# tiems90/mosaic

Hardware: AMD Instinct MI355X
Metric: PIP-join points/sec (H3 res 9) at 1/2/4/8 GPUs + achieved HBM GB/s (higher is better)
Workload: dtype f64

## Files before the change

mosaic_amd/csrc/kernels.hip:

```cpp
#include <hip/hip_runtime.h>
#include <stdint.h>
#include <type_traits>

#include <map>
#include <mutex>

#define H3T_QUAL static __constant__ const
#include "h3_core.h"
#include "bng_core.h"
#include "pip_core.h"
#include "h3_ring.h"
#include "kernels.h"
#include "raster.h"

namespace mgpu {

#ifndef MGPU_BLOCK
#define MGPU_BLOCK 64
#endif
constexpr int kBlock = MGPU_BLOCK;
constexpr int kItems = 4;
constexpr int kTile = kBlock * kItems;
constexpr int kStreamBlock = 256;
static_assert(kTile <= 1024, "point-in-tile indices are 10 bits");
// ... 813 lines not shown
        const double2 q = s_cand_xy[point_stash<G>() ? (uint32_t)li : c];
        px = q.x;
        py = q.y;
      } else {
        px = a.x[MGPU_PT(li)];
        py = a.y[MGPU_PT(li)];
      }
      const ChipHdr& H = t.chip_hdr[ch];
      const uint32_t strip = H.strip_base + (uint32_t)strip_of(py, H.env[1], H.inv_h, (int)H.n_strips);
      one = H.single_ring != 0;
      fl = H.flags;
      pip::strip_bits(t, strip, one, px, py, sub * MGPU_EDGE_STEP, MGPU_EDGE_STEP << lg, &bnd, &par);
    }
    for (uint32_t o = 1; o < (1u << lg); o <<= 1) {
      bnd |= (uint32_t)__shfl_xor((int)bnd, (int)o);
      par ^= (uint32_t)__shfl_xor((int)par, (int)o);
    }
    if (m < nmix && sub == 0 && pip::strip_verdict(t, ch, one, fl, bnd, par, px, py))
      atomicOr(&s_mask[li], 1u << (pj >> 10));
  } else
#endif
  for (uint32_t m = threadIdx.x; m < nmix; m += kBlock) {
    const uint32_t c = s_mix[m];
    const uint32_t pj = s_cand_pj[c];
    const int li = pj & 1023;
    const uint32_t ch = s_first[li] + (pj >> 10);
    const int64_t p = MGPU_PT(li);
    double px, py;
    if (point_stash<G>() || c < (uint32_t)kStash) {
      const double2 q = s_cand_xy[point_stash<G>() ? (uint32_t)li : c];
      px = q.x;
      py = q.y;
    } else {
      px = a.x[p];
      py = a.y[p];
    }
    bool hit;
    if (SLOW && (t.chip_hdr[ch].flags & kChipNoStrips)) {
      hit = pip::chip_locate(t, ch, px, py) == pip::kInterior;
    } else {
#ifdef MGPU_STATS
      uint32_t ne = 0;
      hit = pip::chip_contains_mixed(t, ch, px, py, &ne);
      st_edges += ne;
#else
      hit = pip::chip_contains_mixed(t, ch, px, py);
#endif
    }
    if (hit) atomicOr(&s_mask[li], 1u << (pj >> 10));
  }
  }
#ifdef MGPU_STATS
  if (threadIdx.x == 0) {
    atomicAdd(&a.counters[8], (unsigned long long)s_nmix);
  }
  atomicAdd(&a.counters[9], (unsigned long long)st_edges);
#endif
  __syncthreads();

  MGPU_STAMP(3);
  if (G) {
    uint64_t v[kItems];
    uint32_t mine[kItems];
#pragma unroll
    for (int k = 0; k < kItems; k++) {
      const uint32_t li = threadIdx.x + k * kBlock;
      v[k] = 0;
      mine[k] = 0;
      if (li < gcount) {
        const uint32_t m = s_mask[li];
        v[k] = (uint64_t)s_first[li] | ((uint64_t)m << 32);
        if (a.poly_answers && m && !(m & (m - 1)))
          v[k] = (uint64_t)(uint32_t)t.chip_poly[s_first[li] + __builtin_ctz(m)] | (1ull << 32);
        mine[k] = __popc(m);
      }
    }
#pragma unroll
    for (int k = 0; k < kItems; k++) {
      const uint32_t li = threadIdx.x + k * kBlock;
      if (li < gcount) a.mixed_res[lbase + li] = v[k];
    }
    if (G == 1 && a.in_chunk_pairs) {
      const int lane = threadIdx.x & 63;
      const uint32_t s0 = 4u * (uint32_t)lane;
      const uint4 mq = *(const uint4*)(s_mask + s0);
      const uint32_t mv[4] = {mq.x, mq.y, mq.z, mq.w};
      uint32_t c[4], loc[4], nn[4];
#pragma unroll
      for (int i = 0; i < 4; i++) {
        const bool act = s0 + i < gcount;
        c[i] = act ? ckp[i] / (uint32_t)kChunk : 0xFFFFFFFFu;
        nn[i] = act ? (uint32_t)__popc(mv[i]) : 0u;
        loc[i] = (i ? loc[i - 1] : 0u) + nn[i];
      }
      const uint32_t lane_excl = wave_incl_scan(loc[3]) - loc[3];
      const uint32_t prev_c = __shfl_up(c[3], 1, 64), next_c = __shfl_down(c[0], 1, 64);
      bool head[4];
      uint32_t hpre = 0;
#pragma unroll
      for (int i = 0; i < 4; i++) {
        head[i] = c[i] != 0xFFFFFFFFu && (i ? c[i] != c[i - 1] : (lane == 0 || prev_c != c[0]));
        if (head[i]) hpre = lane_excl + loc[i] - nn[i];
      }
      const unsigned long long hl = __ballot(head[0] || head[1] || head[2] || head[3]);
      const unsigned long long lower = hl & ((1ull << lane) - 1ull);
      uint32_t start = __shfl(hpre, lower ? 63 - __clzll(lower) : 0, 64);
#pragma unroll
      for (int i = 0; i < 4; i++) {
        if (head[i]) start = lane_excl + loc[i] - nn[i];
        const bool tail = c[i] != 0xFFFFFFFFu && (i < 3 ? c[i + 1] != c[i] : (lane == 63 || next_c != c[3]));
        const uint32_t run = lane_excl + loc[i] - start;
        if (tail && run) atomicAdd(&a.in_chunk_pairs[c[i]], run);
      }
    }
    uint32_t tm = 0;
#pragma unroll
    for (int k = 0; k < kItems; k++) tm += mine[k];
    const unsigned long long tot = wave_sum_u64(tm);
    if ((threadIdx.x & 63) == 0 && tot) atomicAdd(&a.group_sum[chunk], (uint32_t)tot);
    return;
  }
  const int l0 = threadIdx.x * kItems;
  uint32_t mine = 0;
#pragma unroll
  for (int k = 0; k < kItems; k++) {
    const int li = l0 + k;
    mine += __popc(s_mask[li]);
    const uint32_t cnt = s_cnt[li];
    if (SLOW && cnt > (uint32_t)kMaskBits) {
      const int64_t p = MGPU_PT(li);
      const Range r{s_first[li], cnt, 0};
      for (uint32_t j = kMaskBits; j < cnt; j++)
        mine += (chip_is_core(t, r, j) || pip::chip_contains_strips(t, r.first + j, a.x[p], a.y[p])) ? 1 : 0;
    }
  }
  const int lane = threadIdx.x & 63, wave = threadIdx.x >> 6;
  uint32_t incl = wave_incl_scan(mine);
  if (lane == 63) s_wave_tot[wave] = incl;
  __syncthreads();
  uint32_t wave_off = 0, agg = 0;
#pragma unroll
  for (int w = 0; w < kBlock / 64; w++) {
    uint32_t v = s_wave_tot[w];
    if (w < wave) wave_off += v;
    agg += v;
  }
  const uint32_t excl = wave_off + incl - mine;

  __shared__ uint64_t s_dst;
  if (threadIdx.x == 0) {
    uint64_t dst = (uint64_t)tile * kSlot;
    if (agg > (uint32_t)kSlot) {
      const unsigned long long off = atomicAdd(a.pool_used, (unsigned long long)agg);
      dst = off + agg <= (unsigned long long)a.pool_cap ? (uint64_t)a.n_tiles * kSlot + off : kNoDst;
    }
    a.tile_count[tile] = agg;
    a.tile_where[tile] = dst;
    if (agg) atomicAdd(&a.group_sum[tile / kScanGroup], agg);
    s_dst = dst;
  }
  const bool staged = agg <= (uint32_t)kOutCap;
  __syncthreads();
  const uint64_t dst = s_dst;
  uint64_t* const rec = dst == kNoDst ? nullptr : a.recs + dst;

  uint32_t pos = excl;
#pragma unroll 1
  for (int k = 0; k < kItems; k++) {
    const int li = l0 + k;
    if (!SLOW) {
      const uint32_t first = s_first[li];
      for (uint32_t m = s_mask[li]; m; m &= m - 1) {
        const int32_t poly = t.chip_poly[first + __builtin_ctz(m)];
        if (staged) {
          s_out_poly[pos] = poly;
          s_out_li[pos] = (uint16_t)li;
        } else if (rec) {
          rec[pos] = ((uint64_t)li << 32) | (uint32_t)poly;
        }
        pos++;
      }
      continue;
    }
    const uint32_t cnt = s_cnt[li];
    if (!cnt) continue;
    const uint32_t first = s_first[li];
    const int64_t p = MGPU_PT(li);
    uint32_t m = s_mask[li];
    const uint32_t nj = cnt < (uint32_t)kMaskBits ? cnt : (uint32_t)kMaskBits;
    for (uint32_t j = 0; j < cnt; j++) {
      bool hit;
      if (!SLOW || j < nj) {
        hit = (m >> j) & 1;
      } else {
        const Range r{first, cnt, 0};
        hit = chip_is_core(t, r, j) || pip::chip_contains_strips(t, first + j, a.x[p], a.y[p]);
      }
      if (!hit) continue;
      const int32_t poly = t.chip_poly[first + j];
      if (staged) {
        s_out_poly[pos] = poly;
        s_out_li[pos] = (uint16_t)li;
      } else if (rec) {
        rec[pos] = ((uint64_t)li << 32) | (uint32_t)poly;
      }
      pos++;
    }
  }
  MGPU_STAMP(4);
  if (!staged || !rec) return;
  __syncthreads();
#ifndef MGPU_NT_RECS
#define MGPU_NT_RECS 1
#endif
  for (uint32_t i = threadIdx.x; i < agg; i += kBlock) {
    const uint64_t v = ((uint64_t)s_out_li[i] << 32) | (uint32_t)s_out_poly[i];
#if MGPU_NT_RECS
    __builtin_nontemporal_store(v, &rec[i]);
#else
    rec[i] = v;
#endif
  }
  MGPU_STAMP(4);
}

#ifndef MGPU_WAVES_PER_EU
#define MGPU_WAVES_PER_EU 8
#endif
#if MGPU_WAVES_PER_EU
#define MGPU_JOIN_ATTR __attribute__((amdgpu_waves_per_eu(MGPU_WAVES_PER_EU)))
#else
#define MGPU_JOIN_ATTR
#endif
template <int IS>
__global__ __launch_bounds__(kBlock) MGPU_JOIN_ATTR void pip_join_kernel(JoinArgs a) {
  join_tile<IS, false>(a, blockIdx.x);
}

template <int IS>
__global__ __launch_bounds__(kBlock) void pip_fix_kernel(JoinArgs a) {
  const uint32_t nd = *a.n_dirty;
  for (uint32_t q = blockIdx.x; q < nd; q += gridDim.x) {
    join_tile<IS, true>(a, a.dirty[q]);
    __syncthreads();
  }
}

#ifndef MGPU_CLS_BLOCK
#define MGPU_CLS_BLOCK 256
#endif
constexpr int kClsBlock = MGPU_CLS_BLOCK;
constexpr int kClsItems = kChunk / kClsBlock;
static_assert(kClsItems * (kClsBlock / 64) == 64, "one wave scans a chunk's ballots");
constexpr uint32_t kCodeMixed32 = 0xFFFFFFFFu;

template <int IS>
struct CodeOf {
  using T = uint16_t;
};
template <>
struct CodeOf<MGPU_BNG> {
  using T = uint32_t;
};


__device__ __forceinline__ uint32_t bng_grid_class(const JoinArgs& a, int64_t p, double px, double py, bool* ok,
                                                     uint32_t* first) {
  const ChipTableView& t = a.chips;
  bool tie = false;
  uint32_t gi = kNoEntry;
  Range r = chip_probe<MGPU_BNG, false>(a, p, px, py, ok, &tie, &gi);
  if (!*ok) return kPixEmpty;
  uint64_t e = 0;
  if (gi != kNoEntry) {
    e = t.grid[gi];
    r = grid_range(e, t.cell_ans_row != nullptr);
  }
  *first = r.first;
  if (r.count == 0) return kPixEmpty;
  if (r.count <= 8 && (r.core & ((1u << r.count) - 1u)) == (1u << r.count) - 1u) return (1u << r.count) - 1u;
  if (t.cell_ans_row && (e & kCellAnsFlag)) {
    const uint32_t eI = (uint32_t)bng::d2i(px), nI = (uint32_t)bng::d2i(py), ed = t.bng_edge;
    const uint32_t col = div_fix(eI, ed, t.bng_inv_edge), row = div_fix(nI, ed, t.bng_inv_edge);
    const uint32_t u = div_fix(eI - col * ed, t.cell_ans_sw, t.cell_ans_inv_sw);
    const uint32_t v = div_fix(nI - row * ed, t.cell_ans_sw, t.cell_ans_inv_sw);
    const uint32_t ai = t.cell_ans_row[row - (uint32_t)t.dense[0].b0] + cell_ans_index(e);
    const uint16_t m = t.cell_ans[((size_t)ai * t.cell_ans_g + v) * t.cell_ans_g + u];
    if (m != kCellAnsMixed && m < 256u) return m;
  }
  return kPixMixed;
}

#ifndef MGPU_CFY_BLOCK
#define MGPU_CFY_BLOCK 512
#endif
constexpr int kCfyBlock = MGPU_CFY_BLOCK;
#ifndef MGPU_CFY_BATCH
#define MGPU_CFY_BATCH 4
#endif
#ifndef MGPU_CFY_WAVES
#define MGPU_CFY_WAVES 1
#endif
constexpr int kCfyBatch = MGPU_CFY_BATCH;
template <int IS>
__global__ __launch_bounds__(kCfyBlock) __attribute__((amdgpu_waves_per_eu(MGPU_CFY_WAVES))) void classify_wave_kernel(SplitArgs sa, int64_t n_chunks) {
  using Code = typename CodeOf<IS>::T;
  constexpr int kW = kCfyBlock / 64;
  constexpr int kItems = kChunk / 64;
  static_assert(kItems % kCfyBatch == 0, "MGPU_CFY_BATCH must divide the points per lane of a chunk");
  const JoinArgs& a = sa.j;
  const ChipTableView& t = a.chips;
  extern __shared__ uint16_t s_blk[];
  const int lane = threadIdx.x & 63, wave = threadIdx.x >> 6;
  const bool use_blk = IS == MGPU_H3 && t.raster_blk != nullptr;
  const bool bng_grid = IS == MGPU_BNG && t.raster_mode == kRasterNone;
  const uint32_t nblk = use_blk ? t.raster_bnx * t.raster_bny : 0u;
  uint32_t* s_band = (uint32_t*)(s_blk + ((nblk + 1) & ~1u));
  if (use_blk)
    for (uint32_t i = threadIdx.x; i < nblk; i += kCfyBlock) s_blk[i] = t.raster_blk[i];
  if (IS == MGPU_H3)
    for (uint32_t i = threadIdx.x; i < t.raster_nband; i += kCfyBlock) s_band[i] = t.raster_band[i];
  __syncthreads();
  Code* codes = (Code*)sa.codes;
  const unsigned long long below = (1ull << lane) - 1ull;
  bool any_bad = false;
  const int64_t ch_step = (int64_t)gridDim.x * kW;
  double bx[kCfyBatch], by[kCfyBatch];
  auto load_batch = [&](int64_t ch, int b, double* X, double* Y) {
#pragma unroll
    for (int k = 0; k < kCfyBatch; k++) {
      const int64_t p = ch * kChunk + (int64_t)(b + k) * 64 + lane;
      X[k] = Y[k] = 0.0;
      if (ch < n_chunks && p < a.n) {
        X[k] = __builtin_nontemporal_load(&a.x[p]);
        Y[k] = __builtin_nontemporal_load(&a.y[p]);
      }
    }
  };
  for (int64_t ch = (int64_t)blockIdx.x * kW + wave; ch < n_chunks; ch += ch_step) {
    const int64_t c0 = ch * kChunk;
    uint32_t pairs = 0, nmixed = 0;
    for (int b = 0; b < kItems; b += kCfyBatch) {
      load_batch(ch, b, bx, by);
      uint32_t ri[kCfyBatch], gix[kCfyBatch], sb[kCfyBatch], bi[kCfyBatch];
#pragma unroll
      for (int k = 0; k < kCfyBatch; k++) {
        ri[k] = kNoPixel;
        gix[k] = 0;
        sb[k] = 0;
        bi[k] = kNoPixel;
        const int64_t pk = c0 + (int64_t)(b + k) * 64 + lane;
        if (pk < a.n && pt_valid(a.valid, a.valid_off, pk)) {
          bool ok = true;
          uint32_t g_ = 0, s_ = 0, b_ = kNoPixel;
          if (IS == MGPU_BNG && bng_grid) {
            const uint32_t m = bng_grid_class(a, pk, bx[k], by[k], &ok, &g_);
            ri[k] = m == kPixMixed ? kRasterFull : m;
          } else {
            ri[k] = raster_index<IS>(t, bx[k], by[k], &ok, &g_, &s_, &b_);
          }
          gix[k] = g_;
          sb[k] = s_;
          bi[k] = use_blk ? b_ : kNoPixel;
          any_bad |= !ok;
        }
      }
      uint32_t cl[kCfyBatch];
      uint64_t ge[kCfyBatch];
#ifndef MGPU_CFY_ABLATE
#define MGPU_CFY_ABLATE 0
#endif
#pragma unroll
      for (int k = 0; k < kCfyBatch; k++) {
#if MGPU_CFY_ABLATE == 1
        cl[k] = ri[k] < kRasterFull ? (ri[k] & 1) : kPixEmpty;
#elif MGPU_CFY_ABLATE == 2
        cl[k] = ri[k] < kRasterFull && bi[k] != kNoPixel && s_blk[bi[k]] != kPixMixed ? s_blk[bi[k]] : kPixEmpty;
#elif MGPU_CFY_ABLATE == 3
        cl[k] = ri[k] < kRasterFull ? (bi[k] != kNoPixel && s_blk[bi[k]] != kPixMixed ? s_blk[bi[k]] : t.raster[ri[k]])
                                    : kPixEmpty;
#elif MGPU_CFY_ABLATE == 4
        cl[k] = ri[k] < kRasterFull ? t.raster[ri[k]] : kPixEmpty;
#elif MGPU_CFY_ABLATE == 5
        cl[k] = ri[k] < kRasterFull ? (bi[k] != kNoPixel && s_blk[bi[k]] != kPixMixed ? s_blk[bi[k]] : kPixMixed)
                                    : kPixEmpty;
#else
        if (IS == MGPU_BNG && bng_grid)
          cl[k] = ri[k] == kRasterFull ? kPixMixed : (ri[k] == kNoPixel ? kPixEmpty : ri[k]);
        else
          cl[k] = ri[k] < kRasterFull ? raster_class_blk(t, s_blk, ri[k], bi[k], sb[k], s_band)
                                      : (ri[k] == kRasterFull ? kPixMixed : kPixEmpty);
#endif
        if (IS == MGPU_BNG && bng_grid) ge[k] = gix[k];
        else ge[k] = (IS == MGPU_BNG && ri[k] < kRasterFull) ? t.grid[gix[k]] : 0ull;
      }
#pragma unroll
      for (int k = 0; k < kCfyBatch; k++) {
        const int64_t p = c0 + (int64_t)(b + k) * 64 + lane;
        const bool valid = p < a.n;
        bool mixed = cl[k] == kPixMixed;
        Code code;
        if (IS == MGPU_H3) {
          code = (Code)cl[k];
          if (!mixed && cl[k] != kPixEmpty) {
            const uint32_t c = cl[k];
            pairs += c < t.raster_pc[0] ? 1u : c < t.raster_pc[1] ? 2u : c < t.raster_pc[2] ? 3u : c < t.raster_pc[3] ? 4u
                     : (uint32_t)__popc((uint32_t)(t.raster_cls[c] >> 32));
          }
        } else {
          const uint32_t first = (uint32_t)ge[k], m = cl[k];
          if (!mixed && m && !(m < 256u && first < (1u << 24))) mixed = true;
          code = (Code)(mixed ? kCodeMixed32 : (m ? (first << 8) | m : 0u));
          if (!mixed) pairs += __popc(m);
        }
        if (valid) MGPU_ST_INTER(code, &codes[p]);
        mixed = mixed && valid;
        const unsigned long long bal = __ballot(mixed);
        if (mixed) sa.mixed_idx[c0 + nmixed + (uint32_t)__popcll(bal & below)] = (uint16_t)((b + k) * 64 + lane);
        nmixed += (uint32_t)__popcll(bal);
      }
    }
    pairs = wave_sum_u32(pairs);
    if (lane == 0) {
      sa.chunk_pairs[ch] = pairs;
      sa.chunk_mixed[ch] = nmixed;
      a.group_cand[ch] = 0;
    }
  }
  count_wave(&a.counters[2], any_bad);
}


#ifndef MGPU_CFY_PAIR
#define MGPU_CFY_PAIR 1
#endif
typedef double dbl2_t __attribute__((ext_vector_type(2)));
template <int IS>
__global__ __launch_bounds__(kCfyBlock) __attribute__((amdgpu_waves_per_eu(MGPU_CFY_WAVES))) void classify_pair_kernel(SplitArgs sa, int64_t n_chunks) {
  using Code = typename CodeOf<IS>::T;
  constexpr int kW = kCfyBlock / 64;
  constexpr int kPairItems = kChunk / 128;
  constexpr int kPB = kCfyBatch / 2 > 0 ? kCfyBatch / 2 : 1;
  constexpr int kPts = 2 * kPB;
  static_assert(kPairItems % kPB == 0, "MGPU_CFY_BATCH / 2 must divide the pair items per lane of a chunk");
  const JoinArgs& a = sa.j;
  const ChipTableView& t = a.chips;
  extern __shared__ uint16_t s_blk[];
  const int lane = threadIdx.x & 63, wave = threadIdx.x >> 6;
  const bool use_blk = IS == MGPU_H3 && t.raster_blk != nullptr;
  const bool bng_grid = IS == MGPU_BNG && t.raster_mode == kRasterNone;
  const uint32_t nblk = use_blk ? t.raster_bnx * t.raster_bny : 0u;
  uint32_t* s_band = (uint32_t*)(s_blk + ((nblk + 1) & ~1u));
  if (use_blk)
    for (uint32_t i = threadIdx.x; i < nblk; i += kCfyBlock) s_blk[i] = t.raster_blk[i];
  if (IS == MGPU_H3)
    for (uint32_t i = threadIdx.x; i < t.raster_nband; i += kCfyBlock) s_band[i] = t.raster_band[i];
  __syncthreads();
  Code* codes = (Code*)sa.codes;
  const unsigned long long below = (1ull << lane) - 1ull;
  bool any_bad = false;
  const int64_t ch_step = (int64_t)gridDim.x * kW;
  for (int64_t ch = (int64_t)blockIdx.x * kW + wave; ch < n_chunks; ch += ch_step) {
    const int64_t c0 = ch * kChunk;
    uint32_t pairs = 0, nmixed = 0;
    for (int b = 0; b < kPairItems; b += kPB) {
      double X[kPts], Y[kPts];
#pragma unroll
      for (int k = 0; k < kPB; k++) {
        const int64_t p = c0 + (int64_t)(b + k) * 128 + 2 * lane;
        if (p + 1 < a.n) {
          const dbl2_t vx = __builtin_nontemporal_load((const dbl2_t*)(a.x + p));
          const dbl2_t vy = __builtin_nontemporal_load((const dbl2_t*)(a.y + p));
          X[2 * k] = vx.x, X[2 * k + 1] = vx.y, Y[2 * k] = vy.x, Y[2 * k + 1] = vy.y;
        } else {
          X[2 * k] = Y[2 * k] = X[2 * k + 1] = Y[2 * k + 1] = 0.0;
          if (p < a.n) X[2 * k] = a.x[p], Y[2 * k] = a.y[p];
        }
      }
      uint32_t ri[kPts], gix[kPts], sb[kPts], bi[kPts];
#pragma unroll
      for (int j = 0; j < kPts; j++) {
        ri[j] = kNoPixel;
        gix[j] = 0;
        sb[j] = 0;
        bi[j] = kNoPixel;
        const int64_t pj = c0 + (int64_t)(b + j / 2) * 128 + 2 * lane + (j & 1);
        if (pj < a.n && pt_valid(a.valid, a.valid_off, pj)) {
          bool ok = true;
          uint32_t g_ = 0, s_ = 0, b_ = kNoPixel;
          if (IS == MGPU_BNG && bng_grid) {
            const uint32_t m = bng_grid_class(a, pj, X[j], Y[j], &ok, &g_);
            ri[j] = m == kPixMixed ? kRasterFull : m;
          } else {
            ri[j] = raster_index<IS>(t, X[j], Y[j], &ok, &g_, &s_, &b_);
          }
          gix[j] = g_;
          sb[j] = s_;
          bi[j] = use_blk ? b_ : kNoPixel;
          any_bad |= !ok;
        }
      }
      uint32_t cl[kPts];
      uint64_t ge[kPts];
#pragma unroll
      for (int j = 0; j < kPts; j++) {
        if (IS == MGPU_BNG && bng_grid) {
          cl[j] = ri[j] == kRasterFull ? kPixMixed : (ri[j] == kNoPixel ? kPixEmpty : ri[j]);
          ge[j] = gix[j];
        } else {
          cl[j] = ri[j] < kRasterFull ? raster_class_blk(t, s_blk, ri[j], bi[j], sb[j], s_band)
                                      : (ri[j] == kRasterFull ? kPixMixed : kPixEmpty);
          ge[j] = (IS == MGPU_BNG && ri[j] < kRasterFull) ? t.grid[gix[j]] : 0ull;
        }
      }
      Code code[kPts];
      bool mixed[kPts];
#pragma unroll
      for (int j = 0; j < kPts; j++) {
        const int64_t pj = c0 + (int64_t)(b + j / 2) * 128 + 2 * lane + (j & 1);
        bool m = cl[j] == kPixMixed;
        if (IS == MGPU_H3) {
          code[j] = (Code)cl[j];
          if (!m && cl[j] != kPixEmpty) {
            const uint32_t c = cl[j];
            pairs += c < t.raster_pc[0] ? 1u : c < t.raster_pc[1] ? 2u : c < t.raster_pc[2] ? 3u : c < t.raster_pc[3] ? 4u
                     : (uint32_t)__popc((uint32_t)(t.raster_cls[c] >> 32));
          }
        } else {
          const uint32_t first = (uint32_t)ge[j], mm = cl[j];
          if (!m && mm && !(mm < 256u && first < (1u << 24))) m = true;
          code[j] = (Code)(m ? kCodeMixed32 : (mm ? (first << 8) | mm : 0u));
          if (!m) pairs += __popc(mm);
        }
        mixed[j] = m && pj < a.n;
      }
#pragma unroll
      for (int k = 0; k < kPB; k++) {
        const int64_t p = c0 + (int64_t)(b + k) * 128 + 2 * lane;
        if (p + 1 < a.n) {
          if (sizeof(Code) == 2) {
            MGPU_ST_INTER((uint32_t)code[2 * k] | ((uint32_t)code[2 * k + 1] << 16), (uint32_t*)(codes + p));
          } else {
            typedef uint32_t u32x2_t __attribute__((ext_vector_type(2)));
            u32x2_t v;
            v.x = (uint32_t)code[2 * k];
            v.y = (uint32_t)code[2 * k + 1];
            MGPU_ST_INTER(v, (u32x2_t*)(codes + p));
          }
        } else if (p < a.n) {
          MGPU_ST_INTER(code[2 * k], &codes[p]);
        }
        const unsigned long long b0 = __ballot(mixed[2 * k]), b1 = __ballot(mixed[2 * k + 1]);
        const uint32_t r0 = nmixed + (uint32_t)__popcll(b0 & below) + (uint32_t)__popcll(b1 & below);
        const uint16_t li = (uint16_t)((b + k) * 128 + 2 * lane);
        if (mixed[2 * k]) sa.mixed_idx[c0 + r0] = li;
        if (mixed[2 * k + 1]) sa.mixed_idx[c0 + r0 + (mixed[2 * k] ? 1u : 0u)] = (uint16_t)(li + 1);
        nmixed += (uint32_t)(__popcll(b0) + __popcll(b1));
      }
    }
    pairs = wave_sum_u32(pairs);
    if (lane == 0) {
      sa.chunk_pairs[ch] = pairs;
      sa.chunk_mixed[ch] = nmixed;
      a.group_cand[ch] = 0;
    }
  }
  count_wave(&a.counters[2], any_bad);
}

#ifndef MGPU_MIXED_LEAN
#define MGPU_MIXED_LEAN 1
#endif
template <int IS>
__global__ __launch_bounds__(kBlock) MGPU_JOIN_ATTR void pip_mixed_kernel(JoinArgs a) {
  const uint32_t nm = a.chunk_mixed[blockIdx.x];
  if (threadIdx.x == 0 && nm > (uint32_t)kGTile) {
    const uint32_t more = (nm - 1) / kGTile;
    const uint32_t q = atomicAdd(a.n_extra, more);
    for (uint32_t t = 0; t < more; t++) a.extra[q + t] = blockIdx.x * kChunkTiles + 1 + t;
  }
  join_tile<IS, false, 2, MGPU_MIXED_LEAN != 0>(a, blockIdx.x * kChunkTiles);
}

template <int IS>
__global__ __launch_bounds__(kBlock) void pip_mixed_more_kernel(JoinArgs a) {
  const uint32_t n = *a.n_extra;
  for (uint32_t q = blockIdx.x; q < n; q += gridDim.x) {
    join_tile<IS, false, 2>(a, a.extra[q]);
    __syncthreads();
  }
}

template <int IS, int G>
__global__ __launch_bounds__(kBlock) void pip_mixed_fix_kernel(JoinArgs a) {
  const uint32_t nd = *a.n_dirty;
  for (uint32_t q = blockIdx.x; q < nd; q += gridDim.x) {
    join_tile<IS, true, G>(a, a.dirty[q]);
    __syncthreads();
  }
}

#ifndef MGPU_EMIT_LDSBAR
#define MGPU_EMIT_LDSBAR 1
#endif
__device__ __forceinline__ void lds_barrier() {
#if MGPU_EMIT_LDSBAR
  asm volatile("s_waitcnt lgkmcnt(0)\n\ts_barrier" ::: "memory");
#else
  __syncthreads();
#endif
}

__device__ __forceinline__ uint32_t chunk_excl_scan(uint32_t v, uint32_t* s_w, uint32_t* total) {
  const int lane = threadIdx.x & 63, wave = threadIdx.x >> 6;
  const uint32_t incl = wave_incl_scan(v);
  if (lane == 63) s_w[wave] = incl;
  lds_barrier();
  uint32_t before = 0, all = 0;
#pragma unroll
  for (int w = 0; w < kClsBlock / 64; w++) {
    before += w < wave ? s_w[w] : 0u;
    all += s_w[w];
  }
  *total = all;
  return before + incl - v;
}

constexpr int kEmitWin = 2048;
#ifndef MGPU_EMIT_SWZ
#define MGPU_EMIT_SWZ 1
#endif
__device__ __forceinline__ uint32_t emit_swz(uint32_t q) { return MGPU_EMIT_SWZ ? q ^ ((q >> 6) & 63u) : q; }
#ifndef MGPU_EMIT_NT
#define MGPU_EMIT_NT 1
#endif
#ifndef MGPU_EMIT_NT_OTHER
#define MGPU_EMIT_NT_OTHER 0
#endif
#ifndef MGPU_EMIT_WAVES
#define MGPU_EMIT_WAVES 7
#endif
#ifndef MGPU_EMIT_WAVES_BNG
#define MGPU_EMIT_WAVES_BNG 5
#endif
#ifndef MGPU_BIN_EMIT_WAVES
#define MGPU_BIN_EMIT_WAVES 5
#endif
constexpr int kEmitCls = 2048;
constexpr int kEmitMres = 512;
#ifndef MGPU_EMIT_MR
#define MGPU_EMIT_MR 1
#endif
__host__ __device__ inline uint32_t emit_cls_staged(const ChipTableView& t) {
  const uint32_t n = t.raster_ncls < t.raster_pc[0] ? t.raster_ncls : t.raster_pc[0];
  return n < (uint32_t)kEmitCls ? n : (uint32_t)kEmitCls;
}
constexpr int kEmitTrash = 64;
typedef uint32_t __attribute__((may_alias)) lds_u32;
template <int N>
__device__ __forceinline__ void emit_forget(uint32_t (&w)[N]) {
#pragma unroll
  for (int i = 0; i < N; i++) asm volatile("" : "+v"(w[i]));
}
template <int IS>
__global__ __launch_bounds__(kClsBlock) __attribute__((amdgpu_waves_per_eu(IS == MGPU_H3 ? MGPU_EMIT_WAVES : MGPU_EMIT_WAVES_BNG))) void split_emit_kernel(SplitArgs sa) {
  using Code = typename CodeOf<IS>::T;
  constexpr int kWords = kClsItems * (int)sizeof(Code) / 4;
  static_assert(kWords % 4 == 0 && kWords >= 4, "whole 16-byte code loads per thread (MGPU_CLS_BLOCK 256 or 512)");
  const JoinArgs& a = sa.j;
  const ChipTableView& t = a.chips;
  __shared__ uint32_t s_w[2][kClsBlock / 64];
  __shared__ uint32_t s_poly[kEmitWin + kEmitTrash];
  __shared__ uint16_t s_pt[kEmitWin + kEmitTrash];
  __shared__ uint64_t s_mr[MGPU_EMIT_MR ? kEmitMres : 1];
  extern __shared__ int32_t s_cp[];
  if (sa.redo_affected && blockIdx.x < *sa.redo_first && !sa.redo_affected[blockIdx.x]) return;
  const int64_t c0 = (int64_t)blockIdx.x * kChunk;
  const int64_t p0 = c0 + (int64_t)threadIdx.x * kClsItems;
  const Code kMixed = IS == MGPU_H3 ? (Code)kPixMixed : (Code)kCodeMixed32;
  uint32_t cw[kWords];
  if (p0 + kClsItems <= a.n) {
    const uint4* src = (const uint4*)((const Code*)sa.codes + p0);
#pragma unroll
    for (int i = 0; i < kWords / 4; i++) {
      const uint4 v = src[i];
      cw[4 * i] = v.x, cw[4 * i + 1] = v.y, cw[4 * i + 2] = v.z, cw[4 * i + 3] = v.w;
    }
  } else {
#pragma unroll
    for (int i = 0; i < kWords; i++) cw[i] = 0;
    const Code* cs = (const Code*)sa.codes;
    for (int k = 0; k < kClsItems; k++)
      if (p0 + k < a.n) {
        const uint32_t c = cs[p0 + k];
        if (sizeof(Code) == 2)
          cw[k >> 1] |= c << ((k & 1) * 16);
        else
          cw[k] = c;
      }
  }
  uint32_t ncp = 0;
  if (IS == MGPU_H3) {
    ncp = emit_cls_staged(t);
    for (uint32_t i = threadIdx.x; i < ncp; i += kClsBlock) s_cp[i] = t.raster_cls_poly[i];
  }
  constexpr uint32_t kMr = MGPU_EMIT_MR ? (uint32_t)kEmitMres : 0u;
#if MGPU_EMIT_MR
  {
    const uint32_t nm = sa.chunk_mixed[blockIdx.x], nms = nm < kMr ? nm : kMr;
    for (uint32_t i = threadIdx.x; i < nms; i += kClsBlock) {
      const uint64_t v = a.mixed_res[c0 + i];
      const uint32_t m = (uint32_t)(v >> 32);
      s_mr[i] = __popc(m) == 1 ? (uint64_t)(uint32_t)t.chip_poly[(uint32_t)v + __builtin_ctz(m)] | (1ull << 32) : v;
    }
  }
#endif
  auto code = [&](int k) -> Code {
    return sizeof(Code) == 2 ? (Code)(cw[k >> 1] >> ((k & 1) * 16)) : (Code)cw[k];
  };
  auto pure = [&](Code c) -> uint64_t {
    if (IS == MGPU_H3) return t.raster_cls[(uint32_t)c];
    return (uint64_t)((uint32_t)c >> 8) | ((uint64_t)((uint32_t)c & 0xFFu) << 32);
  };
  auto mres = [&](uint32_t r) -> uint64_t { return r < kMr ? s_mr[r] : a.mixed_res[c0 + r]; };
  uint32_t nmix = 0;
#pragma unroll
  for (int k = 0; k < kClsItems; k++) nmix += code(k) == kMixed;
  uint32_t all_mixed;
  const uint32_t rank0 = chunk_excl_scan(nmix, s_w[0], &all_mixed);
  uint32_t npair = 0, r = rank0;
  uint32_t emits = 0;
  bool wave_slow = true;
  if constexpr (IS == MGPU_H3) {
    uint32_t cmax = 0, pmax = 0;
    emit_forget(cw);
#pragma unroll
    for (int k = 0; k < kClsItems; k++) {
      const uint32_t c = code(k);
      const bool mixed = c == (uint32_t)kMixed;
      const uint32_t rs = kMr ? (r < kMr - 1 ? r : kMr - 1) : 0u;
      const uint32_t pm = (uint32_t)__popc((uint32_t)(s_mr[rs] >> 32));
      const uint32_t cnt = mixed ? pm : (uint32_t)(c != 0);
      pmax = mixed && pm > pmax ? pm : pmax;
      cmax = !mixed && c > cmax ? c : cmax;
      npair += cnt;
      emits |= (cnt & 1u) << k;
      r += mixed;
    }
    const bool slow = cmax >= ncp || pmax > 1 || (nmix != 0 && r > kMr);
    wave_slow = __any(slow);
  }
  if (wave_slow) {
    npair = 0, r = rank0;
    emit_forget(cw);
#pragma unroll
    for (int k = 0; k < kClsItems; k++) {
      const Code c = code(k);
      if (c == kMixed)
        npair += __popc((uint32_t)(mres(r++) >> 32));
      else if (c != 0) {
        if (IS == MGPU_H3)
          npair += c < t.raster_pc[0]   ? 1u
                   : c < t.raster_pc[1] ? 2u
                   : c < t.raster_pc[2] ? 3u
                   : c < t.raster_pc[3] ? 4u
                                        : (uint32_t)__popc((uint32_t)(pure(c) >> 32));
        else
          npair += (uint32_t)__popc((uint32_t)c & 0xFFu);
      }
    }
  }
  uint32_t total;
  const uint32_t off0 = chunk_excl_scan(npair, s_w[1], &total);
  total = __builtin_amdgcn_readfirstlane(total);
  const uint64_t base = sa.chunk_off[blockIdx.x];
  auto stage_fast = [&](auto one_win, uint32_t w0) {
    constexpr bool kOneWin = decltype(one_win)::value;
    uint32_t q = off0 - w0;
    r = rank0;
    const uint32_t trash = (uint32_t)kEmitWin + (threadIdx.x & 63u);
    const uint32_t pt0 = threadIdx.x * kClsItems;
    uint32_t em = emits;
    emit_forget(cw);
    asm volatile("" : "+v"(q), "+v"(em));
#pragma unroll
    for (int k = 0; k < kClsItems; k++) {
      const uint32_t c = code(k);
      const bool mixed = c == (uint32_t)kMixed;
      const lds_u32* src = mixed ? (const lds_u32*)&s_mr[r] : (const lds_u32*)&s_cp[c];
      const uint32_t poly = *src;
      const bool e = (em >> k) & 1u;
      const uint32_t slot = e && (kOneWin || q < (uint32_t)kEmitWin) ? emit_swz(q) : trash;
      s_poly[slot] = poly;
      s_pt[slot] = (uint16_t)(pt0 + k);
      q += e;
      r += mixed;
    }
  };
  for (uint32_t w0 = 0; w0 < total; w0 += kEmitWin) {
    if (!wave_slow) {
      if (total <= (uint32_t)kEmitWin)
        stage_fast(std::true_type{}, 0u);
      else if (__any(off0 < w0 + kEmitWin && off0 + npair > w0))
        stage_fast(std::false_type{}, w0);
    } else if (off0 < w0 + kEmitWin && off0 + npair > w0) {
      uint32_t q = off0;
      r = rank0;
      emit_forget(cw);
#pragma unroll
      for (int k = 0; k < kClsItems; k++) {
        const Code c = code(k);
        uint64_t v = 0;
        bool has_one = false;
        int32_t one = 0;
        if (c == kMixed) {
          const uint32_t rr = r++;
          v = mres(rr);
          if (rr < kMr && __popc((uint32_t)(v >> 32)) == 1)
            has_one = true, one = (int32_t)(uint32_t)v, v = 0;
        } else if (IS == MGPU_H3 && c != 0 && (uint32_t)c < ncp)
          has_one = true, one = s_cp[(uint32_t)c];
        else if (c != 0)
          v = pure(c);
        if (has_one) {
          if (q >= w0 && q < w0 + kEmitWin) {
            s_poly[emit_swz(q - w0)] = (uint32_t)one;
            s_pt[emit_swz(q - w0)] = (uint16_t)(threadIdx.x * kClsItems + k);
          }
          q++;
        }
        const uint32_t first = (uint32_t)v;
        for (uint32_t m = (uint32_t)(v >> 32); m; m &= m - 1, q++)
          if (q >= w0 && q < w0 + kEmitWin) {
            s_poly[emit_swz(q - w0)] = (uint32_t)t.chip_poly[first + __builtin_ctz(m)];
            s_pt[emit_swz(q - w0)] = (uint16_t)(threadIdx.x * kClsItems + k);
          }
      }
    }
    lds_barrier();
    const uint32_t cnt = total - w0 < (uint32_t)kEmitWin ? total - w0 : (uint32_t)kEmitWin;
    for (uint32_t i = threadIdx.x; i < cnt; i += kClsBlock) {
      const uint64_t q = base + w0 + i;
      if ((int64_t)q >= sa.capacity) break;
      const int64_t p = c0 + s_pt[emit_swz(i)];
#if MGPU_EMIT_NT
      __builtin_nontemporal_store(sa.point_id ? sa.point_id[p] : sa.id_base + p, &sa.out_point[q]);
      __builtin_nontemporal_store((int32_t)s_poly[emit_swz(i)], &sa.out_poly[q]);
#else
      sa.out_point[q] = sa.point_id ? sa.point_id[p] : sa.id_base + p;
      sa.out_poly[q] = (int32_t)s_poly[emit_swz(i)];
#endif
    }
    lds_barrier();
  }
}

constexpr int kScanBlock = 1024;
constexpr int kScanLds = 24576;
__global__ __launch_bounds__(kScanBlock) void tile_scan_kernel(const uint32_t* __restrict__ gsum,
                                                               const uint32_t* __restrict__ gcand, int64_t ng,
                                                               uint64_t* __restrict__ goff,
                                                               unsigned long long* __restrict__ counters,
                                                               const uint32_t* only_if = nullptr) {
  if (only_if && *only_if == 0) return;
  __shared__ unsigned long long s_w[kScanBlock / 64];
  __shared__ uint32_t s_v[kScanLds + kScanBlock];
  __shared__ unsigned long long s_base[kScanBlock];
  const int lane = threadIdx.x & 63, wave = threadIdx.x >> 6;
  const int64_t per = (ng + kScanBlock - 1) / kScanBlock;
// ... 1327 lines not shown
```

Baseline: 111.4 billion.

## Specialize classify kernels for full chunks, no nulls, and batched staged raster lookups

The classify kernels become templated lambdas dispatched on three compile-time flags: whether the raster tables allow a staged lookup, whether a validity bitmap exists, and whether the chunk is fully in range. This removes per-point bounds and null checks on the common path. A new batched raster classifier issues the block, band, pixel and sub-pixel lookups for all points in a batch level by level, so that independent dependent-load chains overlap instead of running one point at a time. The cost is more template instantiations, larger code and possibly higher register pressure, and the staged path assumes the tables have no palette.

```diff
diff --git a/mosaic_amd/csrc/kernels.hip b/mosaic_amd/csrc/kernels.hip
--- a/mosaic_amd/csrc/kernels.hip
+++ b/mosaic_amd/csrc/kernels.hip
@@ -1139,6 +1139,55 @@
 #define MGPU_CFY_WAVES 1
 #endif
 constexpr int kCfyBatch = MGPU_CFY_BATCH;
+
+template <int N>
+__device__ __forceinline__ void raster_class_batch(const ChipTableView& t, const uint16_t* blk, const uint32_t* band,
+                                                   const uint32_t (&ri)[N], const uint32_t (&bi)[N],
+                                                   const uint32_t (&sub)[N], uint32_t (&cl)[N]) {
+  const uint32_t s2 = t.raster_sub_n * t.raster_sub_n;
+  uint32_t c[N], bb[N], px[N], q[N];
+  bool pix[N], ref[N];
+#pragma unroll
+  for (int k = 0; k < N; k++) {
+    c[k] = blk[bi[k] != kNoPixel ? bi[k] : 0u];
+    bb[k] = band[sub[k] >> 16];
+  }
+#pragma unroll
+  for (int k = 0; k < N; k++) {
+    pix[k] = ri[k] < kRasterFull && (bi[k] == kNoPixel || c[k] == kPixMixed);
+    px[k] = t.raster[pix[k] ? ri[k] : 0u];
+  }
+#pragma unroll
+  for (int k = 0; k < N; k++) {
+    ref[k] = pix[k] && px[k] >= 0x8000u && px[k] != kPixMixed;
+    const uint64_t i = ((uint64_t)bb[k] + (px[k] & 0x7FFFu)) * s2 + (sub[k] & 0xFFFFu);
+    q[k] = t.raster_sub[ref[k] ? i : 0ull];
+  }
+#pragma unroll
+  for (int k = 0; k < N; k++)
+    cl[k] = ri[k] >= kRasterFull ? (ri[k] == kRasterFull ? kPixMixed : kPixEmpty) : ref[k] ? q[k] : pix[k] ? px[k] : c[k];
+}
+
+__device__ __forceinline__ bool cfy_staged(const ChipTableView& t, uint32_t nblk) {
+  return t.raster_blk && nblk && t.raster_band && t.raster_nband && !t.raster_pal && t.raster_sub && t.raster_sub_n &&
+         t.raster_nx && t.raster_ny;
+}
+
+template <int IS, class F>
+__device__ __forceinline__ void cfy_dispatch(bool staged, bool nulls, F& run) {
+  if constexpr (IS == MGPU_H3) {
+    if (staged) {
+      if (nulls) run(std::true_type{}, std::true_type{});
+      else run(std::true_type{}, std::false_type{});
+    } else {
+      if (nulls) run(std::false_type{}, std::true_type{});
+      else run(std::false_type{}, std::false_type{});
+    }
+  } else {
+    run(std::false_type{}, std::true_type{});
+  }
+}
+
 template <int IS>
 __global__ __launch_bounds__(kCfyBlock) __attribute__((amdgpu_waves_per_eu(MGPU_CFY_WAVES))) void classify_wave_kernel(SplitArgs sa, int64_t n_chunks) {
   using Code = typename CodeOf<IS>::T;
@@ -1162,23 +1211,21 @@
   const unsigned long long below = (1ull << lane) - 1ull;
   bool any_bad = false;
   const int64_t ch_step = (int64_t)gridDim.x * kW;
-  double bx[kCfyBatch], by[kCfyBatch];
-  auto load_batch = [&](int64_t ch, int b, double* X, double* Y) {
-#pragma unroll
-    for (int k = 0; k < kCfyBatch; k++) {
-      const int64_t p = ch * kChunk + (int64_t)(b + k) * 64 + lane;
-      X[k] = Y[k] = 0.0;
-      if (ch < n_chunks && p < a.n) {
-        X[k] = __builtin_nontemporal_load(&a.x[p]);
-        Y[k] = __builtin_nontemporal_load(&a.y[p]);
-      }
-    }
-  };
-  for (int64_t ch = (int64_t)blockIdx.x * kW + wave; ch < n_chunks; ch += ch_step) {
+  auto run_chunk = [&](int64_t ch, auto staged_c, auto nulls_c, auto full_c) {
+    constexpr bool kStaged = decltype(staged_c)::value, kNulls = decltype(nulls_c)::value, kFull = decltype(full_c)::value;
     const int64_t c0 = ch * kChunk;
     uint32_t pairs = 0, nmixed = 0;
     for (int b = 0; b < kItems; b += kCfyBatch) {
-      load_batch(ch, b, bx, by);
+      double bx[kCfyBatch], by[kCfyBatch];
+#pragma unroll
+      for (int k = 0; k < kCfyBatch; k++) {
+        const int64_t p = c0 + (int64_t)(b + k) * 64 + lane;
+        bx[k] = by[k] = 0.0;
+        if (kFull || p < a.n) {
+          bx[k] = __builtin_nontemporal_load(&a.x[p]);
+          by[k] = __builtin_nontemporal_load(&a.y[p]);
+        }
+      }
       uint32_t ri[kCfyBatch], gix[kCfyBatch], sb[kCfyBatch], bi[kCfyBatch];
 #pragma unroll
       for (int k = 0; k < kCfyBatch; k++) {
@@ -1187,7 +1234,7 @@
         sb[k] = 0;
         bi[k] = kNoPixel;
         const int64_t pk = c0 + (int64_t)(b + k) * 64 + lane;
-        if (pk < a.n && pt_valid(a.valid, a.valid_off, pk)) {
+        if ((kFull || pk < a.n) && (!kNulls || pt_valid(a.valid, a.valid_off, pk))) {
           bool ok = true;
           uint32_t g_ = 0, s_ = 0, b_ = kNoPixel;
           if (IS == MGPU_BNG && bng_grid) {
@@ -1207,34 +1254,40 @@
 #ifndef MGPU_CFY_ABLATE
 #define MGPU_CFY_ABLATE 0
 #endif
-#pragma unroll
-      for (int k = 0; k < kCfyBatch; k++) {
+      if constexpr (kStaged) {
+        raster_class_batch<kCfyBatch>(t, s_blk, s_band, ri, bi, sb, cl);
+#pragma unroll
+        for (int k = 0; k < kCfyBatch; k++) ge[k] = 0ull;
+      } else {
+#pragma unroll
+        for (int k = 0; k < kCfyBatch; k++) {
 #if MGPU_CFY_ABLATE == 1
-        cl[k] = ri[k] < kRasterFull ? (ri[k] & 1) : kPixEmpty;
+          cl[k] = ri[k] < kRasterFull ? (ri[k] & 1) : kPixEmpty;
 #elif MGPU_CFY_ABLATE == 2
-        cl[k] = ri[k] < kRasterFull && bi[k] != kNoPixel && s_blk[bi[k]] != kPixMixed ? s_blk[bi[k]] : kPixEmpty;
+          cl[k] = ri[k] < kRasterFull && bi[k] != kNoPixel && s_blk[bi[k]] != kPixMixed ? s_blk[bi[k]] : kPixEmpty;
 #elif MGPU_CFY_ABLATE == 3
-        cl[k] = ri[k] < kRasterFull ? (bi[k] != kNoPixel && s_blk[bi[k]] != kPixMixed ? s_blk[bi[k]] : t.raster[ri[k]])
-                                    : kPixEmpty;
+          cl[k] = ri[k] < kRasterFull ? (bi[k] != kNoPixel && s_blk[bi[k]] != kPixMixed ? s_blk[bi[k]] : t.raster[ri[k]])
+                                      : kPixEmpty;
 #elif MGPU_CFY_ABLATE == 4
-        cl[k] = ri[k] < kRasterFull ? t.raster[ri[k]] : kPixEmpty;
+          cl[k] = ri[k] < kRasterFull ? t.raster[ri[k]] : kPixEmpty;
 #elif MGPU_CFY_ABLATE == 5
-        cl[k] = ri[k] < kRasterFull ? (bi[k] != kNoPixel && s_blk[bi[k]] != kPixMixed ? s_blk[bi[k]] : kPixMixed)
-                                    : kPixEmpty;
+          cl[k] = ri[k] < kRasterFull ? (bi[k] != kNoPixel && s_blk[bi[k]] != kPixMixed ? s_blk[bi[k]] : kPixMixed)
+                                      : kPixEmpty;
 #else
-        if (IS == MGPU_BNG && bng_grid)
-          cl[k] = ri[k] == kRasterFull ? kPixMixed : (ri[k] == kNoPixel ? kPixEmpty : ri[k]);
-        else
-          cl[k] = ri[k] < kRasterFull ? raster_class_blk(t, s_blk, ri[k], bi[k], sb[k], s_band)
-                                      : (ri[k] == kRasterFull ? kPixMixed : kPixEmpty);
-#endif
-        if (IS == MGPU_BNG && bng_grid) ge[k] = gix[k];
-        else ge[k] = (IS == MGPU_BNG && ri[k] < kRasterFull) ? t.grid[gix[k]] : 0ull;
+          if (IS == MGPU_BNG && bng_grid)
+            cl[k] = ri[k] == kRasterFull ? kPixMixed : (ri[k] == kNoPixel ? kPixEmpty : ri[k]);
+          else
+            cl[k] = ri[k] < kRasterFull ? raster_class_blk(t, s_blk, ri[k], bi[k], sb[k], s_band)
+                                        : (ri[k] == kRasterFull ? kPixMixed : kPixEmpty);
+#endif
+          if (IS == MGPU_BNG && bng_grid) ge[k] = gix[k];
+          else ge[k] = (IS == MGPU_BNG && ri[k] < kRasterFull) ? t.grid[gix[k]] : 0ull;
+        }
       }
 #pragma unroll
       for (int k = 0; k < kCfyBatch; k++) {
         const int64_t p = c0 + (int64_t)(b + k) * 64 + lane;
-        const bool valid = p < a.n;
+        const bool valid = kFull || p < a.n;
         bool mixed = cl[k] == kPixMixed;
         Code code;
         if (IS == MGPU_H3) {
@@ -1263,7 +1316,17 @@
       sa.chunk_mixed[ch] = nmixed;
       a.group_cand[ch] = 0;
     }
-  }
+  };
+  auto run = [&](auto staged_c, auto nulls_c) {
+    for (int64_t ch = (int64_t)blockIdx.x * kW + wave; ch < n_chunks; ch += ch_step) {
+      if (IS == MGPU_H3 && (ch + 1) * kChunk <= a.n) {
+        if constexpr (IS == MGPU_H3) run_chunk(ch, staged_c, nulls_c, std::true_type{});
+      } else {
+        run_chunk(ch, staged_c, nulls_c, std::false_type{});
+      }
+    }
+  };
+  cfy_dispatch<IS>(cfy_staged(t, nblk), a.valid != nullptr, run);
   count_wave(&a.counters[2], any_bad);
 }
 
@@ -1297,7 +1360,8 @@
   const unsigned long long below = (1ull << lane) - 1ull;
   bool any_bad = false;
   const int64_t ch_step = (int64_t)gridDim.x * kW;
-  for (int64_t ch = (int64_t)blockIdx.x * kW + wave; ch < n_chunks; ch += ch_step) {
+  auto run_chunk = [&](int64_t ch, auto staged_c, auto nulls_c, auto full_c) {
+    constexpr bool kStaged = decltype(staged_c)::value, kNulls = decltype(nulls_c)::value, kFull = decltype(full_c)::value;
     const int64_t c0 = ch * kChunk;
     uint32_t pairs = 0, nmixed = 0;
     for (int b = 0; b < kPairItems; b += kPB) {
@@ -1305,7 +1369,7 @@
 #pragma unroll
       for (int k = 0; k < kPB; k++) {
         const int64_t p = c0 + (int64_t)(b + k) * 128 + 2 * lane;
-        if (p + 1 < a.n) {
+        if (kFull || p + 1 < a.n) {
           const dbl2_t vx = __builtin_nontemporal_load((const dbl2_t*)(a.x + p));
           const dbl2_t vy = __builtin_nontemporal_load((const dbl2_t*)(a.y + p));
           X[2 * k] = vx.x, X[2 * k + 1] = vx.y, Y[2 * k] = vy.x, Y[2 * k + 1] = vy.y;
@@ -1322,7 +1386,7 @@
         sb[j] = 0;
         bi[j] = kNoPixel;
         const int64_t pj = c0 + (int64_t)(b + j / 2) * 128 + 2 * lane + (j & 1);
-        if (pj < a.n && pt_valid(a.valid, a.valid_off, pj)) {
+        if ((kFull || pj < a.n) && (!kNulls || pt_valid(a.valid, a.valid_off, pj))) {
           bool ok = true;
           uint32_t g_ = 0, s_ = 0, b_ = kNoPixel;
           if (IS == MGPU_BNG && bng_grid) {
@@ -1339,15 +1403,21 @@
       }
       uint32_t cl[kPts];
       uint64_t ge[kPts];
-#pragma unroll
-      for (int j = 0; j < kPts; j++) {
-        if (IS == MGPU_BNG && bng_grid) {
-          cl[j] = ri[j] == kRasterFull ? kPixMixed : (ri[j] == kNoPixel ? kPixEmpty : ri[j]);
-          ge[j] = gix[j];
-        } else {
-          cl[j] = ri[j] < kRasterFull ? raster_class_blk(t, s_blk, ri[j], bi[j], sb[j], s_band)
-                                      : (ri[j] == kRasterFull ? kPixMixed : kPixEmpty);
-          ge[j] = (IS == MGPU_BNG && ri[j] < kRasterFull) ? t.grid[gix[j]] : 0ull;
+      if constexpr (kStaged) {
+        raster_class_batch<kPts>(t, s_blk, s_band, ri, bi, sb, cl);
+#pragma unroll
+        for (int j = 0; j < kPts; j++) ge[j] = 0ull;
+      } else {
+#pragma unroll
+        for (int j = 0; j < kPts; j++) {
+          if (IS == MGPU_BNG && bng_grid) {
+            cl[j] = ri[j] == kRasterFull ? kPixMixed : (ri[j] == kNoPixel ? kPixEmpty : ri[j]);
+            ge[j] = gix[j];
+          } else {
+            cl[j] = ri[j] < kRasterFull ? raster_class_blk(t, s_blk, ri[j], bi[j], sb[j], s_band)
+                                        : (ri[j] == kRasterFull ? kPixMixed : kPixEmpty);
+            ge[j] = (IS == MGPU_BNG && ri[j] < kRasterFull) ? t.grid[gix[j]] : 0ull;
+          }
         }
       }
       Code code[kPts];
@@ -1369,12 +1439,12 @@
           code[j] = (Code)(m ? kCodeMixed32 : (mm ? (first << 8) | mm : 0u));
           if (!m) pairs += __popc(mm);
         }
-        mixed[j] = m && pj < a.n;
+        mixed[j] = m && (kFull || pj < a.n);
       }
 #pragma unroll
       for (int k = 0; k < kPB; k++) {
         const int64_t p = c0 + (int64_t)(b + k) * 128 + 2 * lane;
-        if (p + 1 < a.n) {
+        if (kFull || p + 1 < a.n) {
           if (sizeof(Code) == 2) {
             MGPU_ST_INTER((uint32_t)code[2 * k] | ((uint32_t)code[2 * k + 1] << 16), (uint32_t*)(codes + p));
           } else {
@@ -1401,7 +1471,17 @@
       sa.chunk_mixed[ch] = nmixed;
       a.group_cand[ch] = 0;
     }
-  }
+  };
+  auto run = [&](auto staged_c, auto nulls_c) {
+    for (int64_t ch = (int64_t)blockIdx.x * kW + wave; ch < n_chunks; ch += ch_step) {
+      if (IS == MGPU_H3 && (ch + 1) * kChunk <= a.n) {
+        if constexpr (IS == MGPU_H3) run_chunk(ch, staged_c, nulls_c, std::true_type{});
+      } else {
+        run_chunk(ch, staged_c, nulls_c, std::false_type{});
+      }
+    }
+  };
+  cfy_dispatch<IS>(cfy_staged(t, nblk), a.valid != nullptr, run);
   count_wave(&a.counters[2], any_bad);
 }
 
```

After: 114.8 billion, median of 6. 3.1% higher.
